# Patman86/SVT-AV1-Mod-by-Patman

Hardware: AMD Instinct MI355X
Metric: encoded fps (4K 10-bit preset 8) + ME+txfm HBM GB/s vs roofline, 1/2/4/8 GPU (higher is better)
Workload: dtype u8 (ME) / int32 (transform)

## Files before the change

svt-av1-mod-by-patman_amd/csrc/me_frame.hip:

```cpp
#include <cstdio>
#include <cstdlib>
#include <cstring>

#include "common.hpp"
#include "sad_device.hpp"

using namespace svthip;
using namespace svthip::dev;

namespace {

#define NL 2
#define NR 4
#define MAX_SAD_VALUE_ (128 * 128 * 255)
#define MAX_U32_ 0xFFFFFFFFu

constexpr uint32_t ME_HME_WIN_DW = 3200;
constexpr uint32_t ME_WIN_DW     = ME_HME_WIN_DW - 64 * 16 - 256;
constexpr uint32_t fp_pitch_c(uint32_t tw) { return (((tw + 3) >> 2) + 17) | 1u; }
constexpr uint32_t FP_TILE_W = ME_WIN_DW / fp_pitch_c(64) >= 63 + 8 ? 64 : 32;
static_assert(ME_WIN_DW / fp_pitch_c(FP_TILE_W) >= 63 + 8, "full-pel window buffer too small for one tile");

#ifndef SVT_HIP_ME_FP_DIRECT
#define SVT_HIP_ME_FP_DIRECT 1
// ... 1366 lines not shown
        const uint16_t th = p.prune_ref_if_me_sad_dev_bigger_than_th;
        if (th != (uint16_t)~0) {
            const uint64_t best = slots_min(sad);
            if (q.slot && q.ri >= 1 && (sad - best) * 100 > (th * best))
                r.do_ref = 0;
        }
    }
}

template <class LDS>
__device__ void finalize_b64(LDS &L, const Ctx &c) {
    ME_CTX_LOCALS(c);
    const uint32_t b64 = c.b64;
    const SvtHipMeFrameOut &out    = job.out;
    const uint32_t          stored = p.enable_me_16x16 ? (p.enable_me_8x8 ? 85u : 21u) : 5u;
    uint32_t               *o_mv   = out.me_mv_array + (size_t)b64 * stored * p.max_refs;
    uint8_t                *o_cand = out.me_candidate_array + (size_t)b64 * stored * p.max_cand;
    uint8_t                *o_tot  = out.total_me_candidate_index + (size_t)b64 * stored;
    const bool single = p.num_of_ref_pic_to_search[0] == 1 && p.num_of_ref_pic_to_search[1] == 0;
    const bool mrpoff = p.num_of_ref_pic_to_search[0] == 1 && p.num_of_ref_pic_to_search[1] == 1;
    if ((single || mrpoff) && tid < stored)
        o_tot[tid] = 1;
    __syncthreads();
    if (tid < p.max_number_of_pus_per_sb && tid < 85) {
        if (single)
            cand_single_ref(L, p, gs, gm, tid, o_mv, o_cand);
        else if (mrpoff)
            cand_mrp_off(L, p, gs, gm, tid, (uint32_t)nlists, o_mv, o_cand, o_tot);
        else
            cand_general(L, p, gs, gm, tid, (uint32_t)nlists, o_mv, o_cand, o_tot);
    }
    __syncthreads();

    if (tid < 64) {
        const uint32_t e8 = L.me_dist[21 + tid];
        const uint32_t d8 = wave_sum_all(e8);
        const uint32_t d16 = wave_sum_all(tid < 16 ? L.me_dist[5 + tid] : 0u), d32 = wave_sum_all(tid < 4 ? L.me_dist[1 + tid] : 0u);
        const uint64_t mean = d8 / 64;
        const int64_t  dv   = (int64_t)e8 - (int64_t)mean;
        const uint64_t sq   = (uint64_t)(dv * dv);
        const uint32_t lo = wave_sum_all((uint32_t)sq & 0xffffu), mid = wave_sum_all((uint32_t)(sq >> 16) & 0xffffu),
                       hi = wave_sum_all((uint32_t)(sq >> 32) & 0xffffu), top = wave_sum_all((uint32_t)(sq >> 48));
        if (tid == 0) {
            const uint64_t ssq = (uint64_t)lo + ((uint64_t)mid << 16) + ((uint64_t)hi << 32) + ((uint64_t)top << 48);
            const uint32_t d64 = L.me_dist[0];
            const uint32_t pix = b64_w * b64_h;
            out.me_8x8_cost_variance[b64] = (uint32_t)(ssq / 64);
            out.rc_me_distortion[b64]     = p.input_resolution_le_480p ? d8 : d16;
            out.me_64x64_distortion[b64]  = div_small(d64 * 4096u, pix);
            out.me_32x32_distortion[b64]  = div_small(d32 * 4096u, pix);
            out.me_16x16_distortion[b64]  = div_small(d16 * 4096u, pix);
            out.me_8x8_distortion[b64]    = div_small(d8 * 4096u, pix);
        }
    }
    if (tid < NL * NR)
        out.search_results[(size_t)b64 * NL * NR + tid] = (&S.sr[0][0])[tid];
}


#ifdef SVT_HIP_ME_ABLATE
__device__ int g_me_stop = 99;
#define ME_STOP(k)          \
    do {                    \
        if (me_stop == (k)) \
            return;         \
    } while (0)
#else
#define ME_STOP(k) \
    do {           \
    } while (0)
#endif

#ifndef SVT_HIP_ME_WGS
#define SVT_HIP_ME_WGS 8
#endif
template <bool MCTF>
__global__ __launch_bounds__(WG_THREADS, SVT_HIP_ME_WGS) void me_b64_kernel(const SvtHipMeFrameJob *__restrict__ jobs) {
    __shared__ MeLds L;
#ifdef SVT_HIP_ME_PROFILE
    unsigned long long prof_last = wall_clock64();
#endif
    __shared__ SvtHipMeFrameJob sjob;
    for (uint32_t i = threadIdx.x; i < sizeof(SvtHipMeFrameJob) / 4; i += blockDim.x)
        ((uint32_t *)&sjob)[i] = ((const uint32_t *)&jobs[blockIdx.y])[i];
    __syncthreads();
    Ctx c;
    if (!make_ctx(c, sjob, blockIdx.x))
        return;
#ifdef SVT_HIP_ME_ABLATE
    const int me_stop = g_me_stop;
#endif
    ME_CTX_LOCALS(c);
    stage_sources(L, c, 7);
    for (uint32_t i = tid; i < NL * NR * 85; i += blockDim.x) gs[i] = 0, gm[i] = 0;
    init_state_lane0(L, c);
    __syncthreads();
    ME_PHASE(0);
    ME_STOP(0);
    if (p.me_early_exit_th || p.me_safe_limit_zz_th) {
        zz_sad_all(L, c);
        zz_prune_lane0(L, c);
        __syncthreads();
    }
    ME_PHASE(1);
    ME_STOP(1);
    {
        const bool pre = p.prehme_enable, split = nlists == 2 && (p.prehme_l1_early_exit || tl == 0);
        const bool l0 = p.enable_hme_flag && p.enable_hme_level0_flag, l1 = p.enable_hme_flag && p.enable_hme_level1_flag;
        const bool l2 = p.enable_hme_flag && p.enable_hme_level2_flag;
        const bool dep = p.enable_me_sr_adjustment && p.distance_based_hme_resizing && p.reduce_hme_l0_sr_th_min &&
            p.reduce_hme_l0_sr_th_max && nref > 1;
        for (int step = 0; step < 6; step++) {
            if (step == 2) {
                if (pre) {
                    phme_prune_lane0(L, c);
                    __syncthreads();
                }
                ME_PHASE(2);
                ME_STOP(2);
            } else if (step == 4) {
                ME_PHASE(3);
                ME_STOP(3);
            } else if (step == 5) {
                ME_PHASE(4);
                ME_STOP(4);
                if (pre || l0 || l1) {
                    stage_sources(L, c, 1);
                    __syncthreads();
                }
            }
            const bool active = step == 0 ? pre : step == 1 ? (pre && split) : step == 2 ? l0 : step == 3 ? (l0 && dep) : step == 4 ? l1 : l2;
            if (!active)
                continue;
            const int f0 = step == 1 ? R0 : (step == 3 ? 1 : 0);
            const int f1 = step == 0 ? (split ? R0 : nref) : (step == 2 ? (dep ? 1 : nref) : nref);
            SearchArgs a;
            for (int part = 0; part < 2; part++) {
                if (step < 2)
                    prehme_round(L, c, f0, f1, step == 0 || tl > 0, part, a);
                else if (step < 4)
                    hme_l0_round(L, c, f0, f1, part, a);
                else if (step == 4)
                    hme_l1_round(L, c, f0, f1, part, a);
                else
                    hme_l2_round(L, c, f0, f1, part, a);
                if (part == 0 && a.search) {
                    ME_SITE(step < 2 ? 0 : (step < 4 ? 1 : step - 2));
#if SVT_HIP_ME_L1_DIRECT
                    const int direct_rows = step == 4 ? wg_direct_plan(L.sh, a.nd, a.src, a.row_dw, a.bw, a.bh) : -1;
                    if (direct_rows >= 0)
                        wg_direct_search(L.sh, a.nd, (uint32_t)direct_rows, a.src, a.row_dw, a.bh);
                    else
#endif
                    wg_multi_search(L.sh, a.nd, a.src, a.row_dw, a.bw, a.bh, L.win, a.cap);
                }
            }
        }
    }
    ME_PHASE(5);
    ME_STOP(5);
    centre_prune_lane0(L, c);
    __syncthreads();
    ME_PHASE(6);
    ME_STOP(6);
    const bool tf_exit = p.me_mctf && S.sr[0][0].hme_sad < p.tf_me_exit_th;
    if (!tf_exit) {
        const bool prepared = p.me_early_exit_th != 0;
        if (prepared)
            fullpel_prepare_all(L, c);
        bool direct = false;
#if SVT_HIP_ME_FP_DIRECT
        if (prepared)
            direct = fullpel_direct_all(L, c);
#endif
        if (!direct)
            for (int li = 0; li < nlists; ++li)
                for (int ri = 0; ri < p.num_of_ref_pic_to_search[li]; ++ri)
                    if (S.sr[li][ri].do_ref)
                        fullpel_ref(L, c, li, ri, true, prepared);
    }
    ME_PHASE(7);
    ME_STOP(7);
    if (p.me_mctf) {
        if (tid < NL * NR)
            job.out.search_results[(size_t)c.b64 * NL * NR + tid] = (&S.sr[0][0])[tid];
        return;
    }
    if (p.enable_hme_flag && p.enable_me_hme_ref_pruning) {
        me_prune_lane0(L, c);
        __syncthreads();
    }
    ME_PHASE(8);
    finalize_b64(L, c);
    ME_PHASE(10);
}

}

#ifdef SVT_HIP_ME_ABLATE
extern "C" __attribute__((visibility("default"))) int32_t svt_hip_debug_me_stop(int32_t k) {
    SVT_HIP_CHECK(hipDeviceSynchronize());
    const int32_t stop = k & 0xff, skip = k >> 8;
    SVT_HIP_CHECK(hipMemcpyToSymbol(HIP_SYMBOL(g_me_stop), &stop, sizeof(stop)));
    SVT_HIP_CHECK(hipMemcpyToSymbol(HIP_SYMBOL(g_ms_skip), &skip, sizeof(skip)));
    return SVT_HIP_OK;
}
#endif

#ifdef SVT_HIP_ME_PROFILE
extern "C" __attribute__((visibility("default"))) int32_t svt_hip_debug_me_profile(unsigned long long out[32], int32_t reset) {
    SVT_HIP_CHECK(hipDeviceSynchronize());
    SVT_HIP_CHECK(hipMemcpyFromSymbol(out, HIP_SYMBOL(g_me_prof), sizeof(unsigned long long) * 11));
    SVT_HIP_CHECK(hipMemcpyFromSymbol(out + 16, HIP_SYMBOL(g_ms_prof), sizeof(unsigned long long) * 16));
    if (reset) {
        unsigned long long z[16] = {};
        SVT_HIP_CHECK(hipMemcpyToSymbol(HIP_SYMBOL(g_me_prof), z, sizeof(z)));
        SVT_HIP_CHECK(hipMemcpyToSymbol(HIP_SYMBOL(g_ms_prof), z, sizeof(unsigned long long) * 16));
    }
    return SVT_HIP_OK;
}
#endif

extern "C" uint32_t svt_hip_me_b64_count(uint32_t width, uint32_t height) {
    const uint32_t aw = (width + 7u) & ~7u, ah = (height + 7u) & ~7u;
    return ((aw + 63) / 64) * ((ah + 63) / 64);
}

static int32_t validate_job(const SvtHipMeFrameJob &j, uint32_t idx) {
    const SvtHipMeParams &p = j.prm;
    auto bad = [&](const char *what) { return refuse("svt_hip_me_frames: job %u: %s", idx, what); };
    if (p.num_hme_sa_w != 2 || p.num_hme_sa_h != 2)
        return bad("num_hme_sa_w/h must be 2 (as in the reference, motion_estimation.c:1945)");
    if (p.num_of_list_to_search < 1 || p.num_of_list_to_search > 2)
        return bad("num_of_list_to_search must be 1 or 2");
    for (int l = 0; l < 2; l++)
        if (p.num_of_ref_pic_to_search[l] > SVT_HIP_ME_MAX_REF)
            return bad("too many reference pictures");
    if (p.num_of_ref_pic_to_search[0] < 1)
        return bad("list 0 needs at least one reference");
    if (p.max_number_of_pus_per_sb != 85)
        return bad("max_number_of_pus_per_sb must be 85 (SQUARE_PU_COUNT)");
    if (p.max_refs == 0 || p.max_cand == 0)
        return bad("max_refs / max_cand not set");
    if (!j.src.full.buf || !j.src.quarter.buf || !j.src.sixteenth.buf)
        return bad("source pyramid incomplete");
    if (j.src.full.width < 64 || j.src.full.height < 64 || j.src.full.width > 16384 || j.src.full.height > 8704)
        return bad("unsupported picture size");
    if (j.src.full.org_x < 64 || j.src.full.org_y < 64)
        return bad("full-resolution planes need >= 64 samples of padding");
    auto pyramid_ok = [](const SvtHipPyramid8 &y) {
        const SvtHipPlane8 *pl[3] = {&y.full, &y.quarter, &y.sixteenth};
        const uint32_t      pad[3] = {64, 32, 16};
        for (int i = 0; i < 3; i++) {
            if (pl[i]->org_x < pad[i] || pl[i]->org_y < pad[i])
                return false;
            if (pl[i]->width != (y.full.width >> i) || pl[i]->height != (y.full.height >> i))
                return false;
            if (pl[i]->stride < (uint32_t)pl[i]->width + 2u * pl[i]->org_x)
                return false;
        }
        return true;
    };
    if (!pyramid_ok(j.src))
        return bad("source pyramid: decimated planes must be width>>1 / width>>2 with >= 32 / 16 samples of padding and stride >= width + 2 * org_x");
    for (int l = 0; l < p.num_of_list_to_search; l++)
        for (int r = 0; r < p.num_of_ref_pic_to_search[l]; r++) {
            const SvtHipPyramid8 &y = j.ref[l][r];
            if (!y.full.buf || !y.quarter.buf || !y.sixteenth.buf)
                return bad("reference pyramid incomplete");
            if (y.full.width != j.src.full.width || y.full.height != j.src.full.height)
                return bad("reference size differs from the source (scaled references are not supported)");
            if (y.full.org_x < 64 || y.full.org_y < 64)
                return bad("reference planes need >= 64 samples of padding");
            if (!pyramid_ok(y))
                return bad("reference pyramid: decimated planes must be width>>1 / width>>2 with >= 32 / 16 samples of padding and stride >= width + 2 * org_x");
        }
    const void *outs[] = {j.out.best_sad, j.out.best_mv, j.out.search_results, j.out.me_mv_array, j.out.me_candidate_array,
                          j.out.total_me_candidate_index, j.out.me_64x64_distortion, j.out.me_32x32_distortion,
                          j.out.me_16x16_distortion, j.out.me_8x8_distortion, j.out.me_8x8_cost_variance,
                          j.out.rc_me_distortion};
    for (const void *o : outs)
        if (!o)
            return bad("NULL output array");
    return SVT_HIP_OK;
}

extern "C" int32_t svt_hip_me_validate_jobs(const SvtHipMeFrameJob *jobs, uint32_t n_jobs, uint32_t *max_b64_out) {
    if (!jobs || n_jobs == 0 || n_jobs > 65535)
        return refuse("svt_hip_me_frames: bad job count");
    uint32_t max_b64 = 0;
    for (uint32_t i = 0; i < n_jobs; i++) {
        const int32_t rc = validate_job(jobs[i], i);
        if (rc != SVT_HIP_OK)
            return rc;
        const uint32_t nb = svt_hip_me_b64_count(jobs[i].src.full.width, jobs[i].src.full.height);
        max_b64           = nb > max_b64 ? nb : max_b64;
    }
    if (max_b64_out)
        *max_b64_out = max_b64;
    return SVT_HIP_OK;
}

static void launch_me(const SvtHipMeFrameJob *d_jobs, uint32_t n_jobs, uint32_t max_b64, hipStream_t st, bool mctf) {
    if (mctf)
        hipLaunchKernelGGL(me_b64_kernel<true>, dim3((max_b64 + 7) / 8 * 8, n_jobs), dim3(WG_THREADS), 0, st, d_jobs);
    else
        hipLaunchKernelGGL(me_b64_kernel<false>, dim3((max_b64 + 7) / 8 * 8, n_jobs), dim3(WG_THREADS), 0, st, d_jobs);
// ... 53 lines not shown
```

svt-av1-mod-by-patman_amd/csrc/sad_device.hpp:

```cpp
#pragma once

#include <hip/hip_runtime.h>
#include <stdint.h>

namespace svthip {
namespace dev {

constexpr int      WG_THREADS = 256;
constexpr int      MAX_SEARCH = 32;
constexpr uint32_t SEG_ALIGN  = 4;
constexpr uint64_t KEY_NONE   = ((uint64_t)0xffffffu << 32) | 0xffffffffu;
constexpr int      MAX_PASS   = 9;

struct SearchDesc {
    const uint8_t *ref;
    uint32_t       ref_stride;
    uint32_t       raw_stride;
    int32_t        sa_w, sa_h;
    uint32_t       skip;
    uint32_t k;
    uint32_t fast;
    uint32_t nq;
    uint32_t no;
    uint32_t n_srows;
// ... 69 lines not shown
                                             uint32_t rows, uint32_t lanes, uint32_t lid) {
    const uint32_t nch = (pitch + 3) >> 2;
    const uint32_t lg  = nch <= 2 ? 1u : (nch <= 4 ? 2u : (nch <= 8 ? 3u : (nch <= 16 ? 4u : 5u)));
    const uint32_t lpr = 1u << lg, rpi = lanes >> lg;
    const uint32_t c0 = lid & (lpr - 1), r0 = lid >> lg;
    for (uint32_t ch = c0; ch < nch; ch += lpr) {
        const uint32_t  nd = pitch - 4 * ch;
        const uint8_t  *g  = g0 + 16 * ch;
        uint32_t       *w  = w0 + 4 * ch;
        for (uint32_t row = r0; row < rows; row += 2 * rpi) {
            const uint32_t row1 = row + rpi;
            const bool     two  = row1 < rows;
            const u128v    a    = load_u128_any(g + (size_t)sad_mul_u24(row, rstride));
            u128v          b    = {0u, 0u, 0u, 0u};
            if (two)
                b = load_u128_any(g + (size_t)sad_mul_u24(row1, rstride));
            uint32_t *wa = w + sad_mul_u24(row, pitch), *wb = w + sad_mul_u24(row1, pitch);
            wa[0] = a.x;
            if (nd > 1) wa[1] = a.y;
            if (nd > 2) wa[2] = a.z;
            if (nd > 3) wa[3] = a.w;
            if (two) {
                wb[0] = b.x;
                if (nd > 1) wb[1] = b.y;
                if (nd > 2) wb[2] = b.z;
                if (nd > 3) wb[3] = b.w;
            }
        }
    }
}

__device__ __forceinline__ uint32_t fast_div(uint32_t n, uint32_t inv) { return inv ? __umulhi(n, inv) : n; }
__device__ __forceinline__ uint32_t make_inv(uint32_t d) { return d > 1 ? 0xffffffffu / d + 1u : 0u; }
__device__ const uint32_t INV_SMALL[65] = {
    0u, 0u, 0x80000000u, 0x55555556u, 0x40000000u, 0x33333334u, 0x2aaaaaabu, 0x24924925u, 0x20000000u, 0x1c71c71du, 0x1999999au, 0x1745d175u, 0x15555556u,
    0x13b13b14u, 0x12492493u, 0x11111112u, 0x10000000u, 0x0f0f0f10u, 0x0e38e38fu, 0x0d79435fu, 0x0ccccccdu, 0x0c30c30du, 0x0ba2e8bbu, 0x0b21642du, 0x0aaaaaabu,
    0x0a3d70a4u, 0x09d89d8au, 0x097b425fu, 0x0924924au, 0x08d3dcb1u, 0x08888889u, 0x08421085u, 0x08000000u, 0x07c1f07du, 0x07878788u, 0x07507508u, 0x071c71c8u,
    0x06eb3e46u, 0x06bca1b0u, 0x06906907u, 0x06666667u, 0x063e7064u, 0x06186187u, 0x05f417d1u, 0x05d1745eu, 0x05b05b06u, 0x0590b217u, 0x0572620bu, 0x05555556u,
    0x0539782au, 0x051eb852u, 0x05050506u, 0x04ec4ec5u, 0x04d4873fu, 0x04bda130u, 0x04a7904bu, 0x04924925u, 0x047dc120u, 0x0469ee59u, 0x0456c798u, 0x04444445u,
    0x04325c54u, 0x04210843u, 0x04104105u, 0x04000000u};
__device__ __forceinline__ uint32_t make_inv_small(uint32_t d) { return d <= 64 ? INV_SMALL[d] : make_inv(d); }

__device__ __forceinline__ void quad_sad(const uint32_t *__restrict__ w, uint32_t w_row_dw,
                                         const uint32_t *__restrict__ s, uint32_t s_row_dw, uint32_t bw, uint32_t bh,
                                         uint32_t out[4]) {
    const uint32_t nfull = bw >> 2, tail = bw & 3;
    const uint32_t rows_per_flush = nfull ? (64u / nfull ? 64u / nfull : 1u) : 64u;
    const uint32_t tmask          = tail ? ((1u << (8 * tail)) - 1u) : 0u;
    uint32_t       a0 = 0, a1 = 0, a2 = 0, a3 = 0;
    uint64_t       acc = 0;
    uint32_t       since = 0;
    for (uint32_t r = 0; r < bh; r++) {
        const uint32_t *wr = w + r * w_row_dw;
        const uint32_t *sr = s + r * s_row_dw;
        uint32_t        lo = wr[0];
        for (uint32_t i = 0; i < nfull; i++) {
            const uint32_t hi = wr[i + 1];
#ifdef SVT_HIP_NO_QSAD
            a0 = __builtin_amdgcn_sad_u8(lo, sr[i], a0);
            a1 = __builtin_amdgcn_sad_u8(__builtin_amdgcn_alignbyte(hi, lo, 1u), sr[i], a1);
            a2 = __builtin_amdgcn_sad_u8(__builtin_amdgcn_alignbyte(hi, lo, 2u), sr[i], a2);
            a3 = __builtin_amdgcn_sad_u8(__builtin_amdgcn_alignbyte(hi, lo, 3u), sr[i], a3);
#else
            acc = __builtin_amdgcn_qsad_pk_u16_u8(pair64(lo, hi), sr[i], acc);
#endif
            lo = hi;
        }
        if (tail) {
            const uint32_t hi = wr[nfull + 1];
            const uint32_t sv = sr[nfull] & tmask;
            a0 = __builtin_amdgcn_sad_u8(lo & tmask, sv, a0);
            a1 = __builtin_amdgcn_sad_u8(__builtin_amdgcn_alignbyte(hi, lo, 1u) & tmask, sv, a1);
            a2 = __builtin_amdgcn_sad_u8(__builtin_amdgcn_alignbyte(hi, lo, 2u) & tmask, sv, a2);
            a3 = __builtin_amdgcn_sad_u8(__builtin_amdgcn_alignbyte(hi, lo, 3u) & tmask, sv, a3);
        }
        if (++since == rows_per_flush) {
            a0 += (uint32_t)(acc & 0xffff), a1 += (uint32_t)((acc >> 16) & 0xffff);
            a2 += (uint32_t)((acc >> 32) & 0xffff), a3 += (uint32_t)(acc >> 48);
            acc = 0, since = 0;
        }
    }
    a0 += (uint32_t)(acc & 0xffff), a1 += (uint32_t)((acc >> 16) & 0xffff);
    a2 += (uint32_t)((acc >> 32) & 0xffff), a3 += (uint32_t)(acc >> 48);
    out[0] = a0, out[1] = a1, out[2] = a2, out[3] = a3;
}

template <uint32_t BW>
__device__ __forceinline__ void quad_sad_fixed(const uint32_t *__restrict__ w, uint32_t w_row_dw, const uint32_t *__restrict__ s,
                                               uint32_t s_row_dw, uint32_t bh, uint32_t out[4]) {
    constexpr uint32_t NF = BW / 4, FLUSH = 64 / NF;
    uint32_t a0 = 0, a1 = 0, a2 = 0, a3 = 0;
    for (uint32_t r0 = 0; r0 < bh; r0 += FLUSH) {
        uint64_t       acc = 0;
        const uint32_t r1  = r0 + FLUSH < bh ? r0 + FLUSH : bh;
#pragma unroll 1
        for (uint32_t r = r0; r < r1; r++) {
            const uint32_t *wr = w + r * w_row_dw;
            const uint32_t *sr = s + r * s_row_dw;
            uint32_t        d[NF + 1];
#pragma unroll
            for (uint32_t i = 0; i <= NF; i++) d[i] = wr[i];
#pragma unroll
            for (uint32_t i = 0; i < NF; i += 4) {
                const uint4 sv = *(const uint4 *)&sr[i];
                acc = __builtin_amdgcn_qsad_pk_u16_u8(pair64(d[i], d[i + 1]), sv.x, acc);
                acc = __builtin_amdgcn_qsad_pk_u16_u8(pair64(d[i + 1], d[i + 2]), sv.y, acc);
                acc = __builtin_amdgcn_qsad_pk_u16_u8(pair64(d[i + 2], d[i + 3]), sv.z, acc);
                acc = __builtin_amdgcn_qsad_pk_u16_u8(pair64(d[i + 3], d[i + 4]), sv.w, acc);
            }
        }
        a0 += (uint32_t)(acc & 0xffff), a1 += (uint32_t)((acc >> 16) & 0xffff);
        a2 += (uint32_t)((acc >> 32) & 0xffff), a3 += (uint32_t)(acc >> 48);
    }
    out[0] = a0, out[1] = a1, out[2] = a2, out[3] = a3;
}

template <uint32_t BW>
__device__ __forceinline__ void oct_sad_fixed(const uint32_t *__restrict__ w, uint32_t w_row_dw, const uint32_t *__restrict__ s,
                                              uint32_t s_row_dw, uint32_t bh, uint32_t out[8]) {
    constexpr uint32_t NF = BW / 4, FLUSH = 64 / NF;
    uint32_t a[8] = {0, 0, 0, 0, 0, 0, 0, 0};
    for (uint32_t r0 = 0; r0 < bh; r0 += FLUSH) {
        uint64_t       acc_a = 0, acc_b = 0;
        const uint32_t r1    = r0 + FLUSH < bh ? r0 + FLUSH : bh;
#pragma unroll 1
        for (uint32_t r = r0; r < r1; r++) {
            const uint32_t *wr = w + r * w_row_dw;
            const uint32_t *sr = s + r * s_row_dw;
            uint32_t        d[NF + 2];
#pragma unroll
            for (uint32_t i = 0; i <= NF + 1; i++) d[i] = wr[i];
#pragma unroll
            for (uint32_t i = 0; i < NF; i += 4) {
                const uint4 sv = *(const uint4 *)&sr[i];
                acc_a = __builtin_amdgcn_qsad_pk_u16_u8(pair64(d[i], d[i + 1]), sv.x, acc_a);
                acc_b = __builtin_amdgcn_qsad_pk_u16_u8(pair64(d[i + 1], d[i + 2]), sv.x, acc_b);
                acc_a = __builtin_amdgcn_qsad_pk_u16_u8(pair64(d[i + 1], d[i + 2]), sv.y, acc_a);
                acc_b = __builtin_amdgcn_qsad_pk_u16_u8(pair64(d[i + 2], d[i + 3]), sv.y, acc_b);
                acc_a = __builtin_amdgcn_qsad_pk_u16_u8(pair64(d[i + 2], d[i + 3]), sv.z, acc_a);
                acc_b = __builtin_amdgcn_qsad_pk_u16_u8(pair64(d[i + 3], d[i + 4]), sv.z, acc_b);
                acc_a = __builtin_amdgcn_qsad_pk_u16_u8(pair64(d[i + 3], d[i + 4]), sv.w, acc_a);
                acc_b = __builtin_amdgcn_qsad_pk_u16_u8(pair64(d[i + 4], d[i + 5]), sv.w, acc_b);
            }
        }
        a[0] += (uint32_t)(acc_a & 0xffff), a[1] += (uint32_t)((acc_a >> 16) & 0xffff);
        a[2] += (uint32_t)((acc_a >> 32) & 0xffff), a[3] += (uint32_t)(acc_a >> 48);
        a[4] += (uint32_t)(acc_b & 0xffff), a[5] += (uint32_t)((acc_b >> 16) & 0xffff);
        a[6] += (uint32_t)((acc_b >> 32) & 0xffff), a[7] += (uint32_t)(acc_b >> 48);
    }
#pragma unroll
    for (int i = 0; i < 8; i++) out[i] = a[i];
}

__device__ __forceinline__ void search_plan_desc(SearchDesc &d, uint32_t bw, uint32_t bh, uint32_t win_cap_dw) {
    d.fast = 0;
    d.k    = 0;
    if (d.sa_w <= 0 || d.sa_h <= 0) {
        d.n_srows = 0, d.nq = 0, d.no = 0;
        return;
    }
    d.n_srows = d.skip ? (uint32_t)d.sa_h / 2u : (uint32_t)d.sa_h;
    d.nq      = ((uint32_t)d.sa_w + 3u) >> 2;
    d.no      = (d.nq + 1u) >> 1;
    if (d.raw_stride != 0 && bw <= 256) {
        d.k = d.ref_stride == d.raw_stride ? 1u : (d.ref_stride == 2 * d.raw_stride ? 2u : (d.ref_stride % d.raw_stride == 0 ? d.ref_stride / d.raw_stride : 0u));
        if (d.k) {
            d.rows_per_pos = (bh - 1) * d.k + 1;
            d.pitch_dw     = (d.nq + ((bw + 3) >> 2) + 1) | 1u;
            d.fast         = (uint64_t)d.pitch_dw * d.rows_per_pos <= win_cap_dw && win_cap_dw <= 65536u;
            d.inv_no       = make_inv_small(d.no);
        }
    }
}

template <bool ITEMS, class SH> __device__ __forceinline__ uint32_t find_seg(const SH &sh, uint32_t nseg, uint32_t v) {
    uint32_t lo = 0, hi = nseg;
    while (hi - lo > 1) {
        const uint32_t mid = (lo + hi) >> 1;
        const uint32_t b   = ITEMS ? sh.seg[mid].item_base : sh.seg[mid].lds_dw;
        if (v >= b)
            lo = mid;
        else
            hi = mid;
    }
    return lo;
}

template <class SH>
__device__ __forceinline__ void wg_multi_search(SH &sh, uint32_t n, const uint32_t *__restrict__ src,
                                       uint32_t src_row_dw, uint32_t bw, uint32_t bh, uint32_t *__restrict__ win,
                                       uint32_t win_cap_dw) {
    uint32_t tid = threadIdx.x;
    asm volatile("" : "+v"(tid));
    const bool src_aligned = (((uint32_t)(uintptr_t)src) & 15u) == 0 && (src_row_dw & 3u) == 0;
#ifdef SVT_HIP_ME_PROFILE
    unsigned long long ms_last = wall_clock64();
#endif
    if (tid < n) {
        search_plan_desc(sh.desc[tid], bw, bh, win_cap_dw);
        sh.best[tid] = KEY_NONE;
    }
    if (tid == 0) {
        sh.next_d = 0, sh.next_j = 0;
    }
    __syncthreads();

    if (tid < 64) {
        uint32_t need = 0, items = 0, nstage = 0;
        bool     valid = false;
        if (tid < n) {
            const SearchDesc &ds = sh.desc[tid];
            if (ds.fast && ds.n_srows) {
                nstage = (ds.n_srows - 1) * (ds.skip ? 2u : 1u) + ds.rows_per_pos;
                need   = (nstage * ds.pitch_dw + SEG_ALIGN - 1) & ~(SEG_ALIGN - 1);
                items  = ds.n_srows * ds.no;
                valid  = true;
            }
        }
        const bool plan_once = n <= 64 && __ballot(valid && need > win_cap_dw) == 0;
        uint32_t   npass = 0;
        if (plan_once) {
            uint32_t pn = need, pi = items;
#pragma unroll
            for (int off = 1; off < 64; off <<= 1) {
                const uint32_t a = __shfl_up(pn, off, 64), b2 = __shfl_up(pi, off, 64);
                if ((int)tid >= off)
                    pn += a, pi += b2;
            }
            const uint64_t vmask = __ballot(valid);
            const uint32_t total_items = __shfl(pi, 63, 64);
            const uint32_t en = pn - need, ei = pi - items;
            const uint32_t sidx = (uint32_t)__popcll(vmask & ((1ull << tid) - 1ull));
            uint64_t       starts = 0;
            uint32_t       base = 0;
            if (vmask) {
                uint32_t first = (uint32_t)__ffsll((unsigned long long)vmask) - 1u;
                for (;;) {
                    starts |= 1ull << first, npass++;
                    base = __shfl(en, (int)first, 64);
                    const uint64_t over = __ballot(valid && tid > first && pn - base > win_cap_dw);
                    if (!over || npass == (uint32_t)MAX_PASS)
                        break;
                    first = (uint32_t)__ffsll((unsigned long long)over) - 1u;
                }
                if (npass == (uint32_t)MAX_PASS && __ballot(valid && tid > first && pn - base > win_cap_dw))
                    npass = 0;
            }
            if (npass && valid) {
                const uint64_t below = starts & ((2ull << tid) - 1ull);
                const uint32_t mypass = (uint32_t)__popcll(below) - 1u, ps = 63u - (uint32_t)__clzll((unsigned long long)below);
                const uint32_t en0 = __shfl(en, (int)ps, 64), ei0 = __shfl(ei, (int)ps, 64);
                SearchSeg     &sg = sh.seg[sidx];
                sg.d = tid, sg.j0 = 0, sg.nj = sh.desc[tid].n_srows, sg.lds_dw = en - en0, sg.nstage = nstage, sg.item_base = ei - ei0;
                if (tid == ps)
                    sh.pass_seg0[mypass] = (uint8_t)sidx, sh.pass_item0[mypass] = ei;
            }
            if (npass && tid == 0)
                sh.pass_seg0[npass] = (uint8_t)__popcll(vmask), sh.pass_item0[npass] = total_items;
        }
        if (tid == 0)
            sh.npass = npass;
    }
    __syncthreads();
    const uint32_t npass_once = sh.npass;

    for (uint32_t pass = 0;; pass++) {
      uint32_t s0 = 0, nseg, nitems_pass;
      bool     onepass;
      if (npass_once) {
        s0 = sh.pass_seg0[pass], nseg = sh.pass_seg0[pass + 1] - s0, nitems_pass = sh.pass_item0[pass + 1] - sh.pass_item0[pass];
        onepass = pass + 1 == npass_once;
      } else {

        if (tid < 64) {
            const uint32_t d0 = sh.next_d, j0 = sh.next_j;
            uint32_t       need = 0, items = 0, nstage = 0, nj = 0, jstart = 0;
            bool           part = false;
            if (tid >= d0 && tid < n) {
                const SearchDesc &ds = sh.desc[tid];
                jstart               = tid == d0 ? j0 : 0;
                if (ds.fast && ds.n_srows > jstart) {
                    const uint32_t step = ds.skip ? 2u : 1u;
                    nj                  = ds.n_srows - jstart;
                    nstage              = (nj - 1) * step + ds.rows_per_pos;
                    if (tid == d0 && nstage * ds.pitch_dw > win_cap_dw) {
                        nj     = (win_cap_dw / ds.pitch_dw - ds.rows_per_pos) / step + 1;
                        nstage = (nj - 1) * step + ds.rows_per_pos;
                        part   = true;
                    }
                    need  = (nstage * ds.pitch_dw + SEG_ALIGN - 1) & ~(SEG_ALIGN - 1);
                    items = nj * ds.no;
                }
            }
            const bool split = __shfl((int)part, (int)(d0 & 63u), 64) != 0;
            uint32_t   need_in = need, items_in = items, cnt_in = need ? 1u : 0u;
#pragma unroll
            for (int off = 1; off < 64; off <<= 1) {
                const uint32_t a = __shfl_up(need_in, off, 64), b2 = __shfl_up(items_in, off, 64), c = __shfl_up(cnt_in, off, 64);
                if ((int)tid >= off)
                    need_in += a, items_in += b2, cnt_in += c;
            }
            const bool take = tid >= d0 && tid < n && need_in <= win_cap_dw && (!split || tid == d0);
            if (take && need) {
                SearchSeg &sg = sh.seg[cnt_in - 1];
                sg.d = tid, sg.j0 = jstart, sg.nj = nj, sg.lds_dw = need_in - need, sg.nstage = nstage;
                sg.item_base = items_in - items;
            }
            const uint32_t ntake = (uint32_t)__popcll(__ballot(take));
            const uint32_t last = d0 + (ntake ? ntake - 1 : 0);
            const uint32_t t_need = __shfl(need_in, (int)(last & 63u), 64), t_items = __shfl(items_in, (int)(last & 63u), 64),
                           t_cnt = __shfl(cnt_in, (int)(last & 63u), 64);
            const uint32_t nj_d0 = __shfl(nj, (int)(d0 & 63u), 64);
            if (tid == 0) {
                sh.nseg = ntake ? t_cnt : 0, sh.nitems = ntake ? t_items : 0, sh.nstage_dw = ntake ? t_need : 0;
                if (split)
                    sh.next_d = d0, sh.next_j = j0 + nj_d0;
                else
                    sh.next_d = d0 + ntake, sh.next_j = 0;
            }
        }
        __syncthreads();
        onepass = sh.next_d >= n;
        MS_PHASE(0);
        nseg = sh.nseg, nitems_pass = sh.nitems;
      }
        if (nseg == 0)
            break;
        {
            const uint32_t nwv = blockDim.x >> 6;
            const bool     per_wave = nseg >= nwv;
            const uint32_t lanes = per_wave ? 64u : blockDim.x, lid = per_wave ? (tid & 63u) : tid;
            for (uint32_t s = per_wave ? (tid >> 6) : 0u; s < nseg; s += per_wave ? nwv : 1u) {
                const SearchSeg   sg = sh.seg[s0 + s];
                const SearchDesc &ds = sh.desc[sg.d];
                const uint32_t    rstride = ds.raw_stride;
#ifdef SVT_HIP_ME_ABLATE
                if (g_ms_skip & 1)
                    continue;
#endif
                stage_rows16(win + sg.lds_dw, ds.pitch_dw, ds.ref + (size_t)sad_mul_u24(ds.skip ? 2 * sg.j0 + 1 : sg.j0, rstride), rstride,
                             sg.nstage, lanes, lid);
            }
        }
        __syncthreads();
        MS_PHASE(1);
#ifdef SVT_HIP_ME_ABLATE
        const uint32_t nitems = (g_ms_skip & 4) ? 0u : nitems_pass;
#else
        const uint32_t nitems = nitems_pass;
#endif
        uint32_t s = 0;
        for (uint32_t item = tid; item < nitems; item += blockDim.x) {
            while (s + 1 < nseg && item >= sh.seg[s0 + s + 1].item_base) s++;
// ... 59 lines not shown
        const uint8_t *sb   = (const uint8_t *)src;
        uint64_t       key  = KEY_NONE;
        for (uint32_t p = tid; p < npos; p += blockDim.x) {
            const uint32_t j = p / (uint32_t)ds.sa_w, sx = p - j * (uint32_t)ds.sa_w;
            const uint32_t sy = ds.skip ? 2 * j + 1 : j;
            const uint8_t *g  = ds.ref + (size_t)sy * ds.raw_stride + sx;
            uint32_t       sad = 0;
            for (uint32_t r = 0; r < bh; r++)
                for (uint32_t c = 0; c < bw; c++) {
                    const int dv = (int)sb[r * src_row_dw * 4 + c] - (int)g[(size_t)r * ds.ref_stride + c];
                    sad += (uint32_t)(dv < 0 ? -dv : dv);
                }
            const uint64_t kk = ((uint64_t)sad << 32) | ((sy << 16) | sx);
            key               = kk < key ? kk : key;
        }
        if (key < KEY_NONE)
            atomicMin((unsigned long long *)&sh.best[d], (unsigned long long)key);
    }
    __syncthreads();
}

#ifndef SVT_HIP_ME_L1_DIRECT
#define SVT_HIP_ME_L1_DIRECT 1
#endif
#ifdef SVT_HIP_NO_QSAD
#undef SVT_HIP_ME_L1_DIRECT
#define SVT_HIP_ME_L1_DIRECT 0
#endif

__device__ __forceinline__ void oct_row32(const u128v w0, const u128v w1, const u128v w2, const uint32_t *__restrict__ sr,
                                          uint64_t &acc_a, uint64_t &acc_b) {
    const uint32_t d[10] = {w0.x, w0.y, w0.z, w0.w, w1.x, w1.y, w1.z, w1.w, w2.x, w2.y};
#pragma unroll
    for (uint32_t i = 0; i < 8; i += 4) {
        const uint4 sv = *(const uint4 *)&sr[i];
        acc_a = __builtin_amdgcn_qsad_pk_u16_u8(pair64(d[i], d[i + 1]), sv.x, acc_a);
        acc_b = __builtin_amdgcn_qsad_pk_u16_u8(pair64(d[i + 1], d[i + 2]), sv.x, acc_b);
        acc_a = __builtin_amdgcn_qsad_pk_u16_u8(pair64(d[i + 1], d[i + 2]), sv.y, acc_a);
        acc_b = __builtin_amdgcn_qsad_pk_u16_u8(pair64(d[i + 2], d[i + 3]), sv.y, acc_b);
        acc_a = __builtin_amdgcn_qsad_pk_u16_u8(pair64(d[i + 2], d[i + 3]), sv.z, acc_a);
        acc_b = __builtin_amdgcn_qsad_pk_u16_u8(pair64(d[i + 3], d[i + 4]), sv.z, acc_b);
        acc_a = __builtin_amdgcn_qsad_pk_u16_u8(pair64(d[i + 3], d[i + 4]), sv.w, acc_a);
        acc_b = __builtin_amdgcn_qsad_pk_u16_u8(pair64(d[i + 4], d[i + 5]), sv.w, acc_b);
    }
}

struct WinRow {
    u128v a, b, c;
};
__device__ __forceinline__ WinRow load_win_row(const uint8_t *g, bool skip_loads) {
    WinRow w = {{0u, 0u, 0u, 0u}, {0u, 0u, 0u, 0u}, {0u, 0u, 0u, 0u}};
    if (!skip_loads)
        w.a = load_u128_any(g), w.b = load_u128_any(g + 16), w.c = load_u128_any(g + 32);
    return w;
}

template <class SH>
__device__ __forceinline__ int wg_direct_plan(SH &sh, uint32_t n, const uint32_t *__restrict__ src, uint32_t src_row_dw, uint32_t bw,
                                              uint32_t bh) {
    uint32_t tid = threadIdx.x;
    asm volatile("" : "+v"(tid));
    if (bw != 32 || bh > 32 || n > (uint32_t)SH::MAXS || n > 64u || (((uint32_t)(uintptr_t)src) & 15u) != 0 || (src_row_dw & 3u) != 0)
        return -1;
    if (tid < n)
        sh.best[tid] = KEY_NONE;
    __syncthreads();
    const uint32_t lane = tid & 63u;
    uint32_t       rows = 0;
    bool           bad  = false;
    if (lane < n) {
        const SearchDesc &ds = sh.desc[lane];
        if (ds.sa_w > 0 && ds.sa_h > 0) {
            rows = (uint32_t)ds.sa_h;
            bad  = ds.raw_stride == 0 || (ds.ref_stride != ds.raw_stride && ds.ref_stride != 2 * ds.raw_stride) || ds.sa_w > 8 ||
                  ds.sa_h > 4 || ds.skip != 0;
        }
    }
    if (__ballot(bad))
        return -1;
    return __ballot(rows >= 3) ? (__ballot(rows == 4) ? 4 : 3) : (__ballot(rows == 2) ? 2 : (__ballot(rows == 1) ? 1 : 0));
}

__device__ __forceinline__ void direct_walk32(const uint8_t *gp, uint32_t rstep, const uint32_t *__restrict__ sr, uint32_t src_row_dw,
                                              uint32_t nrows, bool no_loads, bool no_sad, uint32_t sad[8]) {
    uint64_t acc_a = 0, acc_b = 0;
#pragma unroll 1
    for (uint32_t r = 0; r < nrows; r++) {
        const WinRow wa = load_win_row(gp, no_loads);
        if (no_sad)
            asm volatile("" ::"v"(wa.a), "v"(wa.b), "v"(wa.c));
        else
            oct_row32(wa.a, wa.b, wa.c, sr, acc_a, acc_b);
        gp += rstep, sr += src_row_dw;
    }
    sad[0] += (uint32_t)(acc_a & 0xffff), sad[1] += (uint32_t)((acc_a >> 16) & 0xffff);
    sad[2] += (uint32_t)((acc_a >> 32) & 0xffff), sad[3] += (uint32_t)(acc_a >> 48);
    sad[4] += (uint32_t)(acc_b & 0xffff), sad[5] += (uint32_t)((acc_b >> 16) & 0xffff);
    sad[6] += (uint32_t)((acc_b >> 32) & 0xffff), sad[7] += (uint32_t)(acc_b >> 48);
}

template <class SH>
__device__ __forceinline__ void wg_direct_search(SH &sh, uint32_t n, uint32_t max_rows, const uint32_t *__restrict__ src,
                                                 uint32_t src_row_dw, uint32_t bh) {
    uint32_t tid = threadIdx.x;
    asm volatile("" : "+v"(tid));
    const uint32_t lg = bh < 4 ? 0u : (bh > 16 ? 2u : 1u);
    const uint32_t rpl = (bh + (1u << lg) - 1u) >> lg, g = tid & ((1u << lg) - 1u);
    const uint32_t rb = g * rpl, nrows = bh > rb ? (bh - rb < rpl ? bh - rb : rpl) : 0u;
    const uint32_t inv = max_rows <= 1 ? 0u : (max_rows == 2 ? 0x80000000u : (max_rows == 3 ? 0x55555556u : 0x40000000u));
#ifdef SVT_HIP_ME_ABLATE
    const int      ms_skip = g_ms_skip;
    const bool     no_loads = ms_skip & 1, no_sad = ms_skip & 2;
    const uint32_t nslots = (ms_skip & 4) ? 0u : n * max_rows;
#else
    constexpr bool no_loads = false, no_sad = false;
    const uint32_t nslots = n * max_rows;
#endif
    for (uint32_t slot = tid >> lg; slot < nslots; slot += (uint32_t)WG_THREADS >> lg) {
        const uint32_t    d = fast_div(slot, inv), j = slot - d * max_rows;
        const SearchDesc &ds = sh.desc[d];
        const int32_t     saw = ds.sa_w;
        if (saw <= 0 || (int32_t)j >= ds.sa_h)
            continue;
        const uint32_t  rstep = ds.ref_stride;
        const uint8_t  *gp = ds.ref + (size_t)(sad_mul_u24(j, ds.raw_stride) + sad_mul_u24(rb, rstep));
        const uint32_t *sr = src + rb * src_row_dw;
        uint32_t        sad[8] = {0, 0, 0, 0, 0, 0, 0, 0};
        direct_walk32(gp, rstep, sr, src_row_dw, nrows, no_loads, no_sad, sad);
        if (lg >= 1) {
#pragma unroll
            for (int i = 0; i < 8; i++) sad[i] += (uint32_t)__builtin_amdgcn_update_dpp(0, (int)sad[i], 0xB1, 0xf, 0xf, true);
        }
        if (lg >= 2) {
#pragma unroll
            for (int i = 0; i < 8; i++) sad[i] += (uint32_t)__builtin_amdgcn_update_dpp(0, (int)sad[i], 0x4E, 0xf, 0xf, true);
        }
        if (no_sad) {
#pragma unroll
            for (int i = 0; i < 8; i++) sad[i] = slot + i;
        }
        if (g == 0) {
            uint32_t kmin = ~0u;
#pragma unroll
            for (uint32_t p = 0; p < 8; p++) {
                const uint32_t k = (int32_t)p < saw ? ((sad[p] << 3) | p) : ~0u;
                kmin             = k < kmin ? k : kmin;
            }
            atomicMin((unsigned long long *)&sh.best[d], ((unsigned long long)(kmin >> 3) << 32) | ((j << 16) | (kmin & 7u)));
        }
    }
    __syncthreads();
}

__device__ __forceinline__ void wg_stage_block(uint32_t *__restrict__ dst, uint32_t row_dw, const uint8_t *__restrict__ g,
                                               uint32_t stride, uint32_t bw, uint32_t bh) {
    const uint32_t total = row_dw * bh;
    for (uint32_t idx = threadIdx.x; idx < total; idx += WG_THREADS) {
        const uint32_t r = idx / row_dw, i = idx - r * row_dw;
        const uint8_t *p = g + (size_t)r * stride + 4 * i;
        uint32_t       v = 0;
#pragma unroll
        for (uint32_t b = 0; b < 4; b++)
            if (4 * i + b < bw)
                v |= (uint32_t)p[b] << (8 * b);
        dst[idx] = v;
    }
}

__device__ __forceinline__ uint32_t wave_sum(uint32_t v) {
#pragma unroll
    for (int off = 32; off > 0; off >>= 1) v += __shfl_down(v, off, 64);
    return v;
}

__device__ __forceinline__ uint32_t wave_sum_all(uint32_t v) {
#pragma unroll
    for (int off = 32; off > 0; off >>= 1) v += __shfl_xor(v, off, 64);
    return v;
}

}
}
```

Baseline: 6324.

## Add direct global-memory SAD path for 16-wide pre-HME and HME level-0 searches

Adds a specialised search path for 16-wide blocks with small search areas (width up to 384, height up to 8, no row skipping) in the pre-HME and HME level-0 steps. These searches read reference pixels straight from global memory with qsad instructions, one item per lane covering eight positions, instead of staging windows into LDS through the generic multi-search. Any remaining descriptors still go through wg_multi_search, which now skips the ones already handled. The aim is to cut LDS staging and the barriers around it for small searches, at the cost of uncoalesced global reads and an extra planning pass with a barrier.

```diff
diff --git a/svt-av1-mod-by-patman_amd/csrc/me_frame.hip b/svt-av1-mod-by-patman_amd/csrc/me_frame.hip
--- a/svt-av1-mod-by-patman_amd/csrc/me_frame.hip
+++ b/svt-av1-mod-by-patman_amd/csrc/me_frame.hip
@@ -1542,7 +1542,18 @@
                         wg_direct_search(L.sh, a.nd, (uint32_t)direct_rows, a.src, a.row_dw, a.bh);
                     else
 #endif
-                    wg_multi_search(L.sh, a.nd, a.src, a.row_dw, a.bw, a.bh, L.win, a.cap);
+                    {
+#if SVT_HIP_ME_S16_DIRECT
+                        const int s16 = step < 4 && ((step < 2 ? 2 : 1) & SVT_HIP_ME_S16_DIRECT) != 0
+                            ? wg_s16_plan(L.sh, a.nd, a.src, a.row_dw, a.bw, a.bh) : -1;
+                        if (s16 >= 0)
+                            wg_s16_search(L.sh, a.src, a.row_dw, a.bh);
+                        if (s16 != 0)
+                            wg_multi_search(L.sh, a.nd, a.src, a.row_dw, a.bw, a.bh, L.win, a.cap, s16 > 0);
+#else
+                        wg_multi_search(L.sh, a.nd, a.src, a.row_dw, a.bw, a.bh, L.win, a.cap);
+#endif
+                    }
                 }
             }
         }
diff --git a/svt-av1-mod-by-patman_amd/csrc/sad_device.hpp b/svt-av1-mod-by-patman_amd/csrc/sad_device.hpp
--- a/svt-av1-mod-by-patman_amd/csrc/sad_device.hpp
+++ b/svt-av1-mod-by-patman_amd/csrc/sad_device.hpp
@@ -245,10 +245,17 @@
     for (int i = 0; i < 8; i++) out[i] = a[i];
 }
 
-__device__ __forceinline__ void search_plan_desc(SearchDesc &d, uint32_t bw, uint32_t bh, uint32_t win_cap_dw) {
+constexpr int32_t S16_MAX_W = 384, S16_MAX_ROWS = 8;
+
+__device__ __forceinline__ bool s16_direct_shape(const SearchDesc &d) {
+    return d.sa_w > 0 && d.sa_h > 0 && d.sa_w <= S16_MAX_W && d.sa_h <= S16_MAX_ROWS && d.skip == 0 && d.raw_stride != 0 &&
+        (d.ref_stride == d.raw_stride || d.ref_stride == 2 * d.raw_stride);
+}
+
+__device__ __forceinline__ void search_plan_desc(SearchDesc &d, uint32_t bw, uint32_t bh, uint32_t win_cap_dw, bool s16 = false) {
     d.fast = 0;
     d.k    = 0;
-    if (d.sa_w <= 0 || d.sa_h <= 0) {
+    if (d.sa_w <= 0 || d.sa_h <= 0 || (s16 && s16_direct_shape(d))) {
         d.n_srows = 0, d.nq = 0, d.no = 0;
         return;
     }
@@ -282,7 +289,7 @@
 template <class SH>
 __device__ __forceinline__ void wg_multi_search(SH &sh, uint32_t n, const uint32_t *__restrict__ src,
                                        uint32_t src_row_dw, uint32_t bw, uint32_t bh, uint32_t *__restrict__ win,
-                                       uint32_t win_cap_dw) {
+                                       uint32_t win_cap_dw, bool s16 = false) {
     uint32_t tid = threadIdx.x;
     asm volatile("" : "+v"(tid));
     const bool src_aligned = (((uint32_t)(uintptr_t)src) & 15u) == 0 && (src_row_dw & 3u) == 0;
@@ -290,8 +297,9 @@
     unsigned long long ms_last = wall_clock64();
 #endif
     if (tid < n) {
-        search_plan_desc(sh.desc[tid], bw, bh, win_cap_dw);
-        sh.best[tid] = KEY_NONE;
+        search_plan_desc(sh.desc[tid], bw, bh, win_cap_dw, s16);
+        if (!s16)
+            sh.best[tid] = KEY_NONE;
     }
     if (tid == 0) {
         sh.next_d = 0, sh.next_j = 0;
@@ -657,6 +665,144 @@
     __syncthreads();
 }
 
+#ifndef SVT_HIP_ME_S16_DIRECT
+#define SVT_HIP_ME_S16_DIRECT 1
+#endif
+#ifdef SVT_HIP_NO_QSAD
+#undef SVT_HIP_ME_S16_DIRECT
+#define SVT_HIP_ME_S16_DIRECT 0
+#endif
+#ifndef SVT_HIP_ME_S16_LG
+#define SVT_HIP_ME_S16_LG 0
+#endif
+
+__device__ __forceinline__ void direct_walk16(const uint8_t *gp, uint32_t rstep, const uint32_t *__restrict__ sr, uint32_t src_row_dw,
+                                              uint32_t nrows, bool no_loads, bool no_sad, uint32_t sad[8]) {
+    uint64_t acc_a = 0, acc_b = 0;
+#pragma unroll 1
+    for (uint32_t r = 0; r < nrows; r++) {
+        u128v v = {0u, 0u, 0u, 0u};
+        u64v  w = {0u, 0u};
+        if (!no_loads)
+            v = load_u128_any(gp), w = load_u64_any(gp + 16);
+        if (no_sad) {
+            asm volatile("" ::"v"(v), "v"(w));
+        } else {
+            const uint4 sv = *(const uint4 *)sr;
+            acc_a = __builtin_amdgcn_qsad_pk_u16_u8(pair64(v.x, v.y), sv.x, acc_a);
+            acc_b = __builtin_amdgcn_qsad_pk_u16_u8(pair64(v.y, v.z), sv.x, acc_b);
+            acc_a = __builtin_amdgcn_qsad_pk_u16_u8(pair64(v.y, v.z), sv.y, acc_a);
+            acc_b = __builtin_amdgcn_qsad_pk_u16_u8(pair64(v.z, v.w), sv.y, acc_b);
+            acc_a = __builtin_amdgcn_qsad_pk_u16_u8(pair64(v.z, v.w), sv.z, acc_a);
+            acc_b = __builtin_amdgcn_qsad_pk_u16_u8(pair64(v.w, w.x), sv.z, acc_b);
+            acc_a = __builtin_amdgcn_qsad_pk_u16_u8(pair64(v.w, w.x), sv.w, acc_a);
+            acc_b = __builtin_amdgcn_qsad_pk_u16_u8(pair64(w.x, w.y), sv.w, acc_b);
+        }
+        gp += rstep, sr += src_row_dw;
+    }
+    sad[0] += (uint32_t)(acc_a & 0xffff), sad[1] += (uint32_t)((acc_a >> 16) & 0xffff);
+    sad[2] += (uint32_t)((acc_a >> 32) & 0xffff), sad[3] += (uint32_t)(acc_a >> 48);
+    sad[4] += (uint32_t)(acc_b & 0xffff), sad[5] += (uint32_t)((acc_b >> 16) & 0xffff);
+    sad[6] += (uint32_t)((acc_b >> 32) & 0xffff), sad[7] += (uint32_t)(acc_b >> 48);
+}
+
+template <class SH>
+__device__ __forceinline__ int wg_s16_plan(SH &sh, uint32_t n, const uint32_t *__restrict__ src, uint32_t src_row_dw, uint32_t bw,
+                                           uint32_t bh) {
+    uint32_t tid = threadIdx.x;
+    asm volatile("" : "+v"(tid));
+    if (bw != 16 || bh > 16 || n > (uint32_t)SH::MAXS || n > 64u || (((uint32_t)(uintptr_t)src) & 15u) != 0 || (src_row_dw & 3u) != 0)
+        return -1;
+    if (tid < 64) {
+        uint32_t items = 0, no = 0;
+        bool     direct = false, rest = false;
+        if (tid < n) {
+            const SearchDesc &ds = sh.desc[tid];
+            direct = s16_direct_shape(ds);
+            rest   = !direct && ds.sa_w > 0 && ds.sa_h > 0;
+            if (direct)
+                no = ((uint32_t)ds.sa_w + 7u) >> 3, items = no * (uint32_t)ds.sa_h;
+            sh.best[tid] = KEY_NONE;
+        }
+        uint32_t pi = items;
+#pragma unroll
+        for (int off = 1; off < 64; off <<= 1) {
+            const uint32_t a = __shfl_up(pi, off, 64);
+            if ((int)tid >= off)
+                pi += a;
+        }
+        const uint64_t dmask = __ballot(direct);
+        const uint32_t total = __shfl(pi, 63, 64);
+        const bool     any_rest = __ballot(rest) != 0;
+        if (direct) {
+            SearchSeg &sg = sh.seg[__popcll(dmask & ((1ull << tid) - 1ull))];
+            sg.d = tid, sg.item_base = pi - items, sg.nj = no, sg.nstage = make_inv_small(no);
+        }
+        if (tid == 0)
+            sh.nseg = (uint32_t)__popcll(dmask), sh.nitems = total, sh.nstage_dw = any_rest ? 1u : 0u;
+    }
+    __syncthreads();
+    return (int)sh.nstage_dw;
+}
+
+template <class SH>
+__device__ __forceinline__ void wg_s16_search(SH &sh, const uint32_t *__restrict__ src, uint32_t src_row_dw, uint32_t bh) {
+    uint32_t tid = threadIdx.x;
+    asm volatile("" : "+v"(tid));
+    const uint32_t nseg = sh.nseg;
+#ifdef SVT_HIP_ME_ABLATE
+    const int      ms_skip = g_ms_skip;
+    const bool     no_loads = ms_skip & 1, no_sad = ms_skip & 2;
+    const uint32_t nitems = (ms_skip & 4) ? 0u : sh.nitems;
+#else
+    constexpr bool no_loads = false, no_sad = false;
+    const uint32_t nitems = sh.nitems;
+#endif
+    if (sh.nitems == 0)
+        return;
+    constexpr uint32_t LG = SVT_HIP_ME_S16_LG;
+    static_assert(LG <= 2, "an item's lanes stay inside a group of four");
+    const uint32_t lg = bh < 4 ? 0u : (bh < 8 && LG > 1 ? 1u : LG);
+    const uint32_t rpl = (bh + (1u << lg) - 1u) >> lg, g = tid & ((1u << lg) - 1u);
+    const uint32_t rb = g * rpl, nrows = bh > rb ? (bh - rb < rpl ? bh - rb : rpl) : 0u;
+    uint32_t s = 0;
+    for (uint32_t item = tid >> lg; item < nitems; item += (uint32_t)WG_THREADS >> lg) {
+        while (s + 1 < nseg && item >= sh.seg[s + 1].item_base) s++;
+        const SearchSeg   sg = sh.seg[s];
+        const SearchDesc &ds = sh.desc[sg.d];
+        const uint32_t    li = item - sg.item_base;
+        const uint32_t    j = fast_div(li, sg.nstage), x0 = 8u * (li - sad_mul_u24(j, sg.nj));
+        const uint32_t    rstep = ds.ref_stride;
+        const uint8_t    *gp = ds.ref + (size_t)(sad_mul_u24(j, ds.raw_stride) + sad_mul_u24(rb, rstep) + x0);
+        const uint32_t   *sr = src + rb * src_row_dw;
+        uint32_t          sad[8] = {0, 0, 0, 0, 0, 0, 0, 0};
+        direct_walk16(gp, rstep, sr, src_row_dw, nrows, no_loads, no_sad, sad);
+        if (lg >= 1) {
+#pragma unroll
+            for (int i = 0; i < 8; i++) sad[i] += (uint32_t)__builtin_amdgcn_update_dpp(0, (int)sad[i], 0xB1, 0xf, 0xf, true);
+        }
+        if (LG >= 2 && lg >= 2) {
+#pragma unroll
+            for (int i = 0; i < 8; i++) sad[i] += (uint32_t)__builtin_amdgcn_update_dpp(0, (int)sad[i], 0x4E, 0xf, 0xf, true);
+        }
+        if (no_sad) {
+#pragma unroll
+            for (int i = 0; i < 8; i++) sad[i] = item + i;
+        }
+        if (g == 0) {
+            const uint32_t nvalid = (uint32_t)ds.sa_w - x0;
+            uint32_t       kmin = ~0u;
+#pragma unroll
+            for (uint32_t p = 0; p < 8; p++) {
+                const uint32_t k = p < nvalid ? ((sad[p] << 3) | p) : ~0u;
+                kmin             = k < kmin ? k : kmin;
+            }
+            atomicMin((unsigned long long *)&sh.best[sg.d], ((unsigned long long)(kmin >> 3) << 32) | ((j << 16) | (x0 + (kmin & 7u))));
+        }
+    }
+    __syncthreads();
+}
+
 __device__ __forceinline__ void wg_stage_block(uint32_t *__restrict__ dst, uint32_t row_dw, const uint8_t *__restrict__ g,
                                                uint32_t stride, uint32_t bw, uint32_t bh) {
     const uint32_t total = row_dw * bh;
```

Result: faster. 6441, median of 6 (+1.9%).
